# husheng876/pytorch_nested-unet

Hardware: AMD Instinct MI355X
Metric: images/sec NestedUNet 96x96 bs=16 train (higher is better)
Workload: dtype bf16; 1 GPU; NestedUNet(num_classes=1, in=3, deep_supervision=False) 96x96 per-GPU batch 16, bf16 storage / fp32 accumulate, BCEDiceLoss, SGD(1e-3, 0.9, wd 1e-4), fwd+loss+iou+bwd+sgd per step (BASELINE.json configs[1]); global_batch=16, parallelism=dp1, hip_graph=True

## Files before the change

### include/nunet_diag.h

```cpp
#ifndef NUNET_DIAG_H
#define NUNET_DIAG_H

#include "nunet.h"

#ifdef __cplusplus
extern "C" {
#endif

int nunet_plan_set_lanes(nunet_plan* p, nunet_stream_t* lanes, int32_t n);
int nunet_plan_stamps_read(nunet_plan* plan, int32_t pass, uint64_t* ticks, int32_t cap, int32_t* n_out, char* labels, int32_t label_bytes);
int nunet_debug_stamp(uint64_t* dst, nunet_stream_t stream);
int nunet_debug_spin(int32_t us, int32_t tag, nunet_stream_t stream);

typedef struct {
  int32_t tile;
  int32_t BM, BN, HPMAX, NT;
  int32_t NI, TH, TW, SH;
  int32_t tilesX, tilesY, tilesG;
  int32_t nCoT;
  int32_t S, nch;
  int32_t items;
  int32_t grid;
  int32_t per_cu;
} nunet_conv_launch_info;
int nunet_conv3x3_launch_info(const nunet_conv_desc* d, nunet_conv_launch_info* out);

typedef struct {
  int32_t A, B;
  int32_t NI, TH, TW, SH;
  int32_t tilesX, tilesY, tilesG;
  int32_t nMT;
  int32_t nCoT, nCiT;
  int32_t ksplit;
  int32_t grid;
} nunet_wgrad_launch_info;
int nunet_conv3x3_wgrad_launch_info(const nunet_wgrad_desc* d, nunet_wgrad_launch_info* out);

#ifdef __cplusplus
}
#endif
#endif
```

### pytorch_nested-unet_amd/_lib.py

```python
import ctypes as C
import os
import subprocess

import torch

_HERE = os.path.dirname(os.path.abspath(__file__))
LIB_PATH = os.environ.get("NUNET_LIB_PATH") or os.path.join(_HERE, "libnunet.so")

F32, BF16, F16 = 0, 1, 2
DTYPES = {"fp32": F32, "float32": F32, "bf16": BF16, "bfloat16": BF16, "fp16": F16, "float16": F16,
          torch.float32: F32, torch.bfloat16: BF16, torch.float16: F16}
TORCH_DTYPE = {F32: torch.float32, BF16: torch.bfloat16, F16: torch.float16}

_vp, _i32, _i64, _u32, _f32, _sz = C.c_void_p, C.c_int32, C.c_int64, C.c_uint32, C.c_float, C.c_size_t
BN_SUM_REPLICAS = 8
FX_WORDS = 2
TF_NONE, TF_BN_RELU, TF_BN_RELU_BWD = 0, 1, 2


def fx_zeros(c, device):
    return torch.zeros(BN_SUM_REPLICAS * 2 * c * FX_WORDS, dtype=torch.int64, device=device)


def fx_decode(buf, c):
# ... 9 lines not shown
    buf[0, :, 0] = hi.to(torch.int64)
    buf[0, :, 1] = lo.to(torch.int64)
    return buf.reshape(-1).to(device)


class ConvDesc(C.Structure):
    _fields_ = [("dtype", _i32), ("N", _i32), ("H", _i32), ("W", _i32),
                ("src0", _vp), ("C0", _i32), ("P0", _i32),
                ("src1", _vp), ("C1", _i32), ("P1", _i32),
                ("wpack", _vp), ("bias", _vp),
                ("dst0", _vp), ("D0", _i32), ("Q0", _i32),
                ("dst1", _vp), ("D1", _i32), ("Q1", _i32),
                ("acc_slot_w", _i32), ("acc0_mask", _u32), ("acc1", _i32),
                ("stats", _vp), ("splitk_ws", _vp), ("splitk_ws_floats", _i64),
                ("bn_y", _vp), ("bn_py", _i32), ("bn_mean_invstd", _vp), ("bn_gamma", _vp), ("bn_beta", _vp), ("bn_sums", _vp),
                ("in_tf", _i32), ("tf_training", _i32), ("tf_y", _vp), ("tf_py", _i32), ("tf_fx", _vp),
                ("tf_gamma", _vp), ("tf_beta", _vp), ("tf_conv_bias", _vp),
                ("tf_running_mean", _vp), ("tf_running_var", _vp), ("tf_nbt", _vp), ("tf_mean_invstd", _vp),
                ("tf_momentum", _f32), ("tf_eps", _f32),
                ("tf_dgamma", _vp), ("tf_dbeta", _vp), ("tf_dbias", _vp), ("tf_store", _vp), ("tf_ps", _i32), ("tile", _i32)]


class WgradDesc(C.Structure):
    _fields_ = [("dtype", _i32), ("N", _i32), ("H", _i32), ("W", _i32),
                ("src0", _vp), ("C0", _i32), ("P0", _i32),
                ("src1", _vp), ("C1", _i32), ("P1", _i32),
                ("dy", _vp), ("Cout", _i32), ("PY", _i32),
                ("dw", _vp), ("slab_stride", _i64), ("max_slabs", _i32), ("target_wgs", _i32), ("dw_floats", _i64), ("item_shape", _i32)]


class ConvLaunchInfo(C.Structure):
    _fields_ = [(k, _i32) for k in ("tile", "BM", "BN", "HPMAX", "NT", "NI", "TH", "TW", "SH", "tilesX", "tilesY", "tilesG",
                                    "nCoT", "S", "nch", "items", "grid", "per_cu")]


class WgradLaunchInfo(C.Structure):
    _fields_ = [(k, _i32) for k in ("A", "B", "NI", "TH", "TW", "SH", "tilesX", "tilesY", "tilesG", "nMT", "nCoT", "nCiT",
                                    "ksplit", "grid")]


class BnFwdDesc(C.Structure):
    _fields_ = [("dtype", _i32), ("N", _i32), ("H", _i32), ("W", _i32), ("C", _i32),
                ("y", _vp), ("PY", _i32),
                ("conv_bias", _vp), ("stats", _vp), ("gamma", _vp), ("beta", _vp),
                ("running_mean", _vp), ("running_var", _vp), ("num_batches_tracked", _vp),
                ("save_mean_invstd", _vp),
                ("training", _i32), ("momentum", _f32), ("eps", _f32),
                ("a", _vp), ("PA", _i32), ("pooled", _vp), ("PP", _i32), ("up", _vp), ("PU", _i32)]


class BnBwdDesc(C.Structure):
    _fields_ = [("dtype", _i32), ("N", _i32), ("H", _i32), ("W", _i32), ("C", _i32),
                ("da", _vp), ("PDA", _i32), ("y", _vp), ("PY", _i32),
                ("mean_invstd", _vp), ("gamma", _vp), ("beta", _vp),
                ("sums", _vp), ("dgamma", _vp), ("dbeta", _vp), ("dbias", _vp),
                ("dy", _vp), ("PDY", _i32)]


class BnrDesc(C.Structure):
    _fields_ = [("y", _vp), ("PY", _i32), ("mean_invstd", _vp), ("gamma", _vp), ("beta", _vp), ("sums", _vp)]


class ProfEntry(C.Structure):
    _fields_ = [("name", C.c_char * 48), ("launches", _i32), ("ms", C.c_double), ("flops", C.c_double),
                ("bytes", C.c_double)]

# ... 64 lines not shown
    "nunet_nchw_to_nhwc": (_i32, [_vp, _i32, _i32, _i32, _i32, _i32, _vp, _i32, _vp]),
    "nunet_plan_create": (_vp, [C.POINTER(PlanCfg)]),
    "nunet_plan_destroy": (None, [_vp]),
    "nunet_plan_arena_bytes": (C.c_size_t, [_vp]),
    "nunet_plan_param_count": (_i64, [_vp]),
    "nunet_plan_bnbuf_count": (_i64, [_vp]),
    "nunet_plan_bn_layers": (_i32, [_vp]),
    "nunet_plan_num_heads": (_i32, [_vp]),
    "nunet_plan_forward": (_i32, [_vp, _vp, _vp, _vp, _vp, _vp, _sz, _vp, _i32, _vp]),
    "nunet_plan_stage_u8": (_i32, [_vp, _vp, _vp, _vp, _vp, _f32, _vp, _sz, _vp]),
    "nunet_plan_backward": (_i32, [_vp, _vp, _vp, _vp, _sz, _vp, _i32, _vp]),
    "nunet_plan_backward_phase": (_i32, [_vp, _vp, _vp, _vp, _sz, _vp, _i32, _i32, _vp]),
    "nunet_plan_grad_scratch": (_i32, [_vp, C.POINTER(_i64), C.POINTER(_i64), C.POINTER(_i64)]),
    "nunet_plan_bucket0_enable": (_i32, [_vp, _i32]),
    "nunet_plan_bucket0_wait": (_i32, [_vp, _vp]),
    "nunet_plan_opt_step": (_i32, [_vp, _vp, C.POINTER(Optim), _vp, _sz, _f32, _vp, _i32, _vp]),
    "nunet_plan_set_inpass_opt": (_i32, [_vp, _vp, C.POINTER(Optim), _f32, _vp]),
    "nunet_plan_grad_sqnorm_ws_bytes": (C.c_size_t, [_vp]),
    "nunet_plan_grad_sqnorm": (_i32, [_vp, _vp, _sz, _vp, _sz, _vp]),
    "nunet_plan_repack": (_i32, [_vp, _vp, _vp, _sz, _vp]),
    "nunet_plan_feature": (_i64, [_vp, _i32, _i32, C.POINTER(_i32), C.POINTER(_i32)]),
    "nunet_plan_set_multistream": (_i32, [_vp, _i32]),
    "nunet_plan_set_schedule": (_i32, [_vp, _i32]),
    "nunet_plan_calibrate": (_i32, [_vp, _i32]),
    "nunet_plan_set_lane_priority": (_i32, [_vp, _i32]),
    "nunet_plan_reset_lanes": (_i32, [_vp]),
    "nunet_plan_set_lanes": (_i32, [_vp, C.POINTER(_vp), _i32]),
    "nunet_profile_begin": (_i32, []),
    "nunet_profile_end": (_i32, [C.POINTER(ProfEntry), _i32, C.POINTER(_i32)]),
    "nunet_debug_spin": (_i32, [_i32, _i32, _vp]),
    "nunet_debug_stamp": (_i32, [_vp, _vp]),
    "nunet_conv3x3_launch_info": (_i32, [C.POINTER(ConvDesc), C.POINTER(ConvLaunchInfo)]),
    "nunet_conv3x3_wgrad_launch_info": (_i32, [C.POINTER(WgradDesc), C.POINTER(WgradLaunchInfo)]),
    "nunet_graph_begin": (_i32, [_vp]),
    "nunet_graph_end": (_i32, [_vp, C.POINTER(_vp)]),
    "nunet_graph_launch": (_i32, [_vp, _vp]),
    "nunet_graph_info": (_i32, [_vp, C.POINTER(_i32), C.POINTER(_i32), C.POINTER(_i32)]),
    "nunet_graph_destroy": (None, [_vp]),
    "nunet_seg_begin": (_i32, [_vp, _i32]),
    "nunet_seg_end": (_i32, [_vp, C.POINTER(_vp)]),
    "nunet_seg_launch": (_i32, [_vp, _vp]),
    "nunet_seg_info": (_i32, [_vp, C.POINTER(_i32), C.POINTER(_i32), C.POINTER(_i32), C.POINTER(_i32)]),
    "nunet_seg_destroy": (None, [_vp]),
    "nunet_plan_stamps_read": (_i32, [_vp, _i32, C.POINTER(C.c_uint64), _i32, C.POINTER(_i32), C.c_char_p, _i32]),
}

_lib = None


class NunetError(RuntimeError):
    pass


def build(verbose=False):
    cmd = ["make", "-C", os.path.join(_HERE, "csrc"), "-j4"]
    r = subprocess.run(cmd, capture_output=True, text=True)
    if r.returncode != 0:
        raise NunetError("building libnunet.so failed:\n" + r.stdout + r.stderr)
    if verbose:
        print(r.stdout)
    return LIB_PATH


def lib():
    global _lib
    if _lib is None:
# ... 54 lines not shown
```

### pytorch_nested-unet_amd/csrc/conv3x3.hip

```cpp
#include <stdlib.h>
#include <type_traits>

#include "common.h"

template <typename T> struct Mma;
template <> struct Mma<bf16_t> {
  typedef bf16x8 Frag;
  static __device__ __forceinline__ Frag load(const bf16_t* p) { return *reinterpret_cast<const bf16x8*>(p); }
  static __device__ __forceinline__ void mma(f32x16& acc, const Frag& a, const Frag& b) {
    acc = __builtin_amdgcn_mfma_f32_32x32x16_bf16(a, b, acc, 0, 0, 0);
  }
  static __device__ __forceinline__ void sink(const Frag& a) { asm volatile("" :: "v"(a)); }
};
template <> struct Mma<f16_t> {
  typedef f16x8 Frag;
  static __device__ __forceinline__ Frag load(const f16_t* p) { return *reinterpret_cast<const f16x8*>(p); }
  static __device__ __forceinline__ void mma(f32x16& acc, const Frag& a, const Frag& b) {
    acc = __builtin_amdgcn_mfma_f32_32x32x16_f16(a, b, acc, 0, 0, 0);
  }
  static __device__ __forceinline__ void sink(const Frag& a) { asm volatile("" :: "v"(a)); }
};
template <> struct Mma<float> {
  struct Frag { f32x4 lo, hi; };
  static __device__ __forceinline__ Frag load(const float* p) {
// ... 111 lines not shown
#define KSTAMP_RT(i) do {} while (0)
#endif

#ifndef NUNET_ABLATE
#define NUNET_ABLATE 0
#endif

static inline int conv_coef_floats(int lt, int cin, bool bnr, int cout) { return (lt == 1 ? 2 : lt == 2 ? 4 : 0) * cin + (bnr ? 4 * cout : 0) + cout; }

struct ConvGroup { int n; int grid[CONV_GROUP_MAX]; ConvP p[CONV_GROUP_MAX]; };

#ifndef NUNET_XCD_REMAP
#define NUNET_XCD_REMAP 1
#endif
__device__ __forceinline__ int xcd_remap(int b, int G) {
  if (!NUNET_XCD_REMAP) return b;
  const int x = b & 7, l = b >> 3, q = G >> 3, rem = G & 7;
  return (x < rem ? x * (q + 1) : rem * (q + 1) + (x - rem) * q) + l;
}
__device__ __forceinline__ void conv_group_decode(const ConvGroup& g, int b, int& k, int& v) {
  int base = 0, prevg = 0, live = g.n;
  k = 0; v = b;
#pragma unroll
  for (int j = 0; j < CONV_GROUP_MAX; ++j) {
    if (j < g.n) {
      const int span = (g.grid[j] - prevg) * live;
      if (b >= base && b < base + span) { const int r = b - base; const int q = r / live; k = j + (r - q * live); v = prevg + q; }
      base += span; prevg = g.grid[j]; --live;
    }
  }
}

template <typename T, int WM, int WN, int SM, int SN, bool SK, bool BNR, int LT>
__global__ __launch_bounds__(64 * WM * WN, 2) void conv3x3_kernel(ConvGroup grp) {
  typedef ConvCfg<T, WM, WN, SM, SN> C;
  int gk = 0, vbid = (int)blockIdx.x;
  if (grp.n > 1) conv_group_decode(grp, (int)blockIdx.x, gk, vbid);
  gk = __builtin_amdgcn_readfirstlane(gk); vbid = __builtin_amdgcn_readfirstlane(vbid);
  const ConvP& p = grp.p[gk];
  const int vgrid = grp.grid[gk];
  typedef Mma<T> M;
  constexpr int PS = C::PS, EPV = C::EPV, BN = C::BN, BM = C::BM, NT = C::NT, KS = C::KS, OS = C::OS;

  __shared__ __attribute__((aligned(16))) T s_buf[C::STAGE_ELEMS];
  __shared__ int s_hidx[BM];
  __shared__ int s_mxy[BM];
  __shared__ int s_hxy[C::HPMAX];
  __shared__ int s_gpix[BM];
  __shared__ float s_red[2 * WM * BN];
  extern __shared__ __attribute__((aligned(16))) float s_coef[];
  T* const s_halo = s_buf;
  T* const s_w = s_buf + C::HALO_ELEMS;
  float* const s_bnc = s_coef + (LT == 1 ? 2 : LT == 2 ? 4 : 0) * p.Cin;
  float* const s_bias = s_bnc + (BNR ? 4 : 0) * p.Cout;

  const int tid = threadIdx.x, lane = tid & 63, wave = tid >> 6;
  const int wm = wave / WN, wn = wave % WN;
  const int r = lane & 31, h = lane >> 5;
  const int HW2 = p.TW + 2, HH2 = p.TH + 2;
  const int HP = p.NI * HH2 * HW2;
  const int THW = p.TH * p.TW;
  KSTAMP(0); KSTAMP_RT(30);
  [[maybe_unused]] int kst = 4;

  for (int m = tid; m < BM; m += NT) {
    const int r32 = m & 31;
    const int q = (r32 < 4) ? r32 : (r32 < 12) ? r32 + 12 : (r32 < 16) ? r32 - 8 : (r32 < 20) ? r32 + 8 : (r32 < 28) ? r32 - 12 : r32;
    const int t = (m & ~31) + q;
    const int ni = fastdiv(t, p.invTHW);
    const int rem = t - ni * THW;
    const int ly = fastdiv(rem, p.invTW), lx = rem - ly * p.TW;
    const bool ok = ni < p.NI;
    s_hidx[m] = ok ? ((ni * HH2 + ly + 1) * HW2 + lx + 1) : (HW2 + 1);
    s_mxy[m] = ok ? ((ni << 20) | (ly << 10) | lx) : -1;
  }
  for (int hp = tid; hp < C::HPMAX; hp += NT) {
    int code = -1;
    if (hp < HP) {
      const int ni = fastdiv(hp, p.invHH2HW2);
      const int rem = hp - ni * (HH2 * HW2);
      const int hy = fastdiv(rem, p.invHW2), hx = rem - hy * HW2;
      code = (ni << 20) | (hy << 10) | hx;
    }
    s_hxy[hp] = code;
  }
  __syncthreads();
  KSTAMP(1);

  int abase[SM];
#pragma unroll
  for (int a = 0; a < SM; ++a) abase[a] = s_hidx[(wm * SM + a) * 32 + r] * PS + 8 * h;
  int toff[9];
#pragma unroll
  for (int tap = 0; tap < 9; ++tap) toff[tap] = ((tap / 3 - 1) * HW2 + (tap % 3 - 1)) * PS;
  const int bbase = ((wn * SN) * 32 + r) * PS + 8 * h;
  int hcode[C::UH];
  unsigned interior = 0u;
#pragma unroll
  for (int k = 0; k < C::UH; ++k) {
    const int hp = (tid + k * NT) >> 2;
    hcode[k] = hp < C::HPMAX ? s_hxy[hp] : -1;
    if (LT != 0 && hcode[k] >= 0) {
      const int hy = (hcode[k] >> 10) & 1023, hx = hcode[k] & 1023;
      if (hy >= 1 && hy <= p.TH && hx >= 1 && hx <= p.TW) interior |= 1u << k;
    }
  }
  const int seg = tid & 3;

  struct Item { int co0, n0, y0, x0, ks; };
  auto decode = [&](int item) {
    Item it;
    it.ks = 0;
    if constexpr (SK) { const int q = fastdiv(item, p.invS); it.ks = item - q * p.S; item = q; }
    int q = fastdiv(item, p.invCoT);
    it.co0 = (item - q * p.nCoT) * BN; item = q;
    q = fastdiv(item, p.invTX);
    it.x0 = (item - q * p.tilesX) * p.TW; item = q;
    q = fastdiv(item, p.invTY);
    it.y0 = (item - q * p.tilesY) * p.TH;
    it.n0 = q * p.NI;
    return it;
  };

  int hgp[C::UH];
  auto set_hgp = [&](const Item& it) {
#pragma unroll
    for (int k = 0; k < C::UH; ++k) {
      int gp = -1;
      if (hcode[k] >= 0) {
        const int n = it.n0 + (hcode[k] >> 20), y = it.y0 + ((hcode[k] >> 10) & 1023) - 1, x = it.x0 + (hcode[k] & 1023) - 1;
        gp = map_pixel(n, y, x, p.N, p.H, p.W, p.SH, p.SHinv);
      }
      hgp[k] = gp;
    }
  };

  Vec16<T> hreg[C::UH];
  Vec16<T> yreg[LT == 2 ? C::UH : 1];
  Vec16<T> wreg[C::UW];
  unsigned woff[C::UW];
#pragma unroll
  for (int k = 0; k < C::UW; ++k) {
    const int u = tid + k * NT;
    const int row = u >> 2;
    const int tap = row / BN, co = row - tap * BN;
    woff[k] = row < 9 * BN ? (unsigned)(((tap * p.Cout + co) * p.Cin + seg * EPV) * (int)sizeof(T)) : (unsigned)(seg * 16);
  }
  unsigned wco = 0u;
  auto set_ptrs = [&](const Item& it) { wco = (unsigned)(it.co0 * p.Cin * (int)sizeof(T)); };
  struct LoadCtx { const char* base; unsigned pb, cb, yb, ycb, wb; };
  auto load_ctx = [&](int kb) {
    LoadCtx c;
    const bool s0 = LT != 0 || kb < p.C0;
    c.base = (const char*)(s0 ? p.src0 : p.src1);
    c.pb = (unsigned)(s0 ? p.P0 : p.P1) * (unsigned)sizeof(T);
    c.cb = (unsigned)((s0 ? kb : kb - p.C0) * (int)sizeof(T) + seg * 16);
    c.yb = (unsigned)p.tf_py * (unsigned)sizeof(T);
    c.ycb = (unsigned)(kb * (int)sizeof(T) + seg * 16);
    c.wb = (unsigned)(kb * (int)sizeof(T)) + wco;
    return c;
  };
  constexpr int NU = C::UH + C::UW;
  auto load_unit = [&](const LoadCtx& c, int u) {
    if (u < C::UH) {
      const unsigned gp = hgp[u] < 0 ? 0u : (unsigned)hgp[u];
      hreg[u].raw = *reinterpret_cast<const u32x4*>(c.base + (gp * c.pb + c.cb));
      if constexpr (LT == 2) yreg[u].raw = *reinterpret_cast<const u32x4*>((const char*)p.tf_y + (gp * c.yb + c.ycb));
    } else {
      wreg[u - C::UH].raw = *reinterpret_cast<const u32x4*>((const char*)p.w + (woff[u - C::UH] + c.wb));
    }
  };
  auto load_regs = [&](int kb) {
    const LoadCtx c = load_ctx(kb);
#pragma unroll
    for (int u = 0; u < NU; ++u) load_unit(c, u);
  };
  auto write_lds = [&](int kb, bool store) {
    if constexpr (LT == 0) {
#pragma unroll
      for (int k = 0; k < C::UH; ++k) {
        const int u = tid + k * NT;
        if ((k + 1) * NT <= C::HPMAX * 4 || (u >> 2) < C::HPMAX) st16(&s_halo[(u >> 2) * PS + seg * EPV], hgp[k] >= 0 ? hreg[k] : zero16<T>());
      }
    } else {
      typedef typename FV<T>::type V;
      const int c0 = kb + seg * EPV;
      const V sc = ldf<T>(&s_coef[c0]), sh = ldf<T>(&s_coef[p.Cin + c0]);
      V cA, cB;
      if constexpr (LT == 2) { cA = ldf<T>(&s_coef[2 * p.Cin + c0]); cB = ldf<T>(&s_coef[3 * p.Cin + c0]); }
#pragma unroll
      for (int k = 0; k < C::UH; ++k) {
        const int u = tid + k * NT;
        if ((k + 1) * NT <= C::HPMAX * 4 || (u >> 2) < C::HPMAX) {
          const bool ok = hgp[k] >= 0;
          V v;
          if constexpr (LT == 1) v = bn_relu_apply<V>(vec_to_f<T>(hreg[k]), sc, sh);
          else v = bn_relu_bwd_apply<V>(vec_to_f<T>(hreg[k]), vec_to_f<T>(yreg[k]), sc, sh, cA, cB);
          Vec16<T> o = vec_from_f<T>(v);
          if (!ok) o = zero16<T>();
          st16(&s_halo[(u >> 2) * PS + seg * EPV], o);
          if (store && ok && ((interior >> k) & 1u)) st16((T*)p.tf_store + (size_t)hgp[k] * p.tf_ps + c0, o);
        }
      }
    }
#pragma unroll
    for (int k = 0; k < C::UW; ++k) {
      const int u = tid + k * NT;
      if ((k + 1) * NT <= 9 * BN * 4 || (u >> 2) < 9 * BN) st16(&s_w[(u >> 2) * PS + seg * EPV], wreg[k]);
    }
  };

  f32x16 acc[SM][SN];
#pragma unroll
  for (int a = 0; a < SM; ++a)
#pragma unroll
    for (int b = 0; b < SN; ++b)
#pragma unroll
      for (int i = 0; i < 16; ++i) acc[a][b][i] = 0.f;

  auto chunk_kb = [&](int c) { return c < p.nch0 ? c * C::KC : p.C0 + (c - p.nch0) * C::KC; };
  constexpr int NSTEP = 9 * KS;
  auto sweep = [&](auto LOADS, const LoadCtx& lc) {
    constexpr bool WITH_LOADS = decltype(LOADS)::value;
    constexpr int PD = 1;
    constexpr int NB = PD + 1;
    typename M::Frag fa[NB][SM], fb[NB][SN];
    auto read_step = [&](int j) {
      const int tap = j / KS, ks = j % KS, bu = j % NB;
#pragma unroll
      for (int a = 0; a < SM; ++a) fa[bu][a] = M::load(&s_halo[abase[a] + toff[tap] + ks * 16]);
#pragma unroll
      for (int b = 0; b < SN; ++b) fb[bu][b] = M::load(&s_w[bbase + (tap * BN + b * 32) * PS + ks * 16]);
    };
#pragma unroll
    for (int j = 0; j < PD; ++j) read_step(j);
#pragma unroll
    for (int j = 0; j < NSTEP; ++j) {
      if (j + PD < NSTEP && !(NUNET_ABLATE & 2)) read_step(j + PD);
      if constexpr (WITH_LOADS && !(NUNET_ABLATE & 4)) {
#pragma unroll
        for (int u = 0; u < NU; ++u)
          if ((u * NSTEP) / NU == j) load_unit(lc, u);
      }
      __builtin_amdgcn_sched_barrier(0);
#pragma unroll
      for (int a = 0; a < SM; ++a)
#pragma unroll
        for (int b = 0; b < SN; ++b) {
          if constexpr (NUNET_ABLATE & 1) { M::sink(fa[j % NB][a]); M::sink(fb[j % NB][b]); }
          else M::mma(acc[a][b], fa[j % NB][a], fb[j % NB][b]);
        }
      __builtin_amdgcn_sched_barrier(0);
    }
  };
  auto epi_sk = [&](const Item& cur) {
    float* slab = p.slabs + (size_t)cur.ks * p.slab_stride;
#pragma unroll
    for (int b = 0; b < SN; ++b) {
      const int co = cur.co0 + (wn * SN + b) * 32 + r;
#pragma unroll
      for (int a = 0; a < SM; ++a) {
#pragma unroll
        for (int i = 0; i < 16; ++i) {
          const int gp = s_gpix[(wm * SM + a) * 32 + acc_row(i, h)];
          if (gp >= 0) slab[(size_t)gp * p.Cout + co] = acc[a][b][i];
          acc[a][b][i] = 0.f;
        }
      }
    }
  };
  static_assert(SM * 16 <= 64, "row-validity mask of the epilogue is one 64-bit word");
  Vec16<T> byv[BNR ? C::UO : 1];
  auto issue_byv = [&](const Item& cur) {
    if constexpr (BNR) {
      constexpr int SEGS = BN / EPV;
      const int sg = tid % SEGS, m0 = tid / SEGS;
#pragma unroll
      for (int k = 0; k < C::UO; ++k) {
        const int m = m0 + k * (NT / SEGS);
        const int gp = m < BM ? s_gpix[m] : -1;
        byv[k] = ld16((const T*)p.bn_y + (size_t)(gp < 0 ? 0 : gp) * p.bn_py + cur.co0 + sg * EPV);
      }
    }
  };
  auto epi_plain = [&](const Item& cur, T* const s_out) {
    constexpr int SEGS = BN / EPV;
    const int sg = tid % SEGS, m0 = tid / SEGS;
    int gpu[C::UO];
#pragma unroll
    for (int k = 0; k < C::UO; ++k) {
      const int m = m0 + k * (NT / SEGS);
      gpu[k] = m < BM ? s_gpix[m] : -1;
    }
    unsigned long long rowmask = 0ull;
    if (p.stats) {
#pragma unroll
      for (int a = 0; a < SM; ++a)
#pragma unroll
        for (int i = 0; i < 16; ++i) rowmask |= (s_gpix[(wm * SM + a) * 32 + acc_row(i, h)] >= 0 ? 1ull : 0ull) << (a * 16 + i);
    }
    KSTAMP(kst); ++kst;
    __syncthreads();
    KSTAMP(kst); ++kst;
#pragma unroll
    for (int b = 0; b < SN; ++b) {
      const int cl = (wn * SN + b) * 32 + r;
      const float bias = s_bias[cur.co0 + cl];
      float s1 = 0.f, s2 = 0.f;
#pragma unroll
      for (int a = 0; a < SM; ++a) {
#pragma unroll
        for (int i = 0; i < 16; ++i) {
          const int m = (wm * SM + a) * 32 + acc_row(i, h);
          const T tv = from_f32<T>(acc[a][b][i] + bias);
          if (!(NUNET_ABLATE & 1024)) s_out[m * OS + cl] = tv;
          const float d = ((rowmask >> (a * 16 + i)) & 1ull) ? to_f32(tv) - bias : 0.f;
          s1 += d; s2 += d * d;
          acc[a][b][i] = 0.f;
        }
      }
      if (p.stats) {
        s1 += __shfl_xor(s1, 32);
        s2 += __shfl_xor(s2, 32);
        if (h == 0) { s_red[(wm * BN + cl) * 2 + 0] = s1; s_red[(wm * BN + cl) * 2 + 1] = s2; }
      }
    }
    KSTAMP(kst); ++kst;
    __syncthreads();
    KSTAMP(kst); ++kst;
    typedef typename FV<T>::type V;
    V bmean, bistd, bsc, bsh, r1 = V(0.f), r2 = V(0.f);
    if constexpr (BNR) {
      const int c0 = cur.co0 + sg * EPV;
      bmean = ldf<T>(&s_bnc[c0]); bistd = ldf<T>(&s_bnc[p.Cout + c0]); bsc = ldf<T>(&s_bnc[2 * p.Cout + c0]); bsh = ldf<T>(&s_bnc[3 * p.Cout + c0]);
    }
    const int co = cur.co0 + sg * EPV;
    const bool to0 = co < p.D0;
    T* const qb = to0 ? (T*)p.dst0 + co : (T*)p.dst1 + (co - p.D0);
    const int qs = to0 ? __builtin_amdgcn_readfirstlane(p.Q0) : __builtin_amdgcn_readfirstlane(p.Q1);
    const bool accum = to0 ? ((p.acc0_mask >> (p.slot_w > 0 ? fastdiv(co, p.inv_slot_w) : 0)) & 1u) != 0u : p.acc1 != 0;
    const bool any_accum = p.acc0_mask != 0u || p.acc1 != 0;
    Vec16<T> vv[C::UO];
#pragma unroll
    for (int k = 0; k < C::UO; ++k) {
      const int m = m0 + k * (NT / SEGS);
      vv[k] = ld16(&s_out[(m < BM ? m : 0) * OS + sg * EPV]);
    }
#pragma unroll
    for (int k = 0; k < C::UO; ++k) {
// ... 54 lines not shown
  Item cur = decode(item);
  set_hgp(cur);
  set_ptrs(cur);
  int cc = 0, c_hi = 0;
  int kb = 0;
  if constexpr (SK) { cc = cur.ks * p.nch / p.S; c_hi = (cur.ks + 1) * p.nch / p.S; kb = chunk_kb(cc); }
  KSTAMP(2);
  load_regs(kb);
  bool first_chunk = true;
  for (int c = tid; c < p.Cout; c += NT) s_bias[c] = p.bias ? p.bias[c] : 0.f;
  if constexpr (BNR) {
    for (int c = tid; c < p.Cout; c += NT) {
      const float mean = p.bn_mi[c], istd = p.bn_mi[p.Cout + c];
      const float sc = p.bn_gamma[c] * istd;
      s_bnc[c] = mean; s_bnc[p.Cout + c] = istd; s_bnc[2 * p.Cout + c] = sc; s_bnc[3 * p.Cout + c] = __builtin_fmaf(-mean, sc, p.bn_beta[c]);
    }
  }
  if constexpr (LT == 1) {
    BnStatArgs a; a.fx = p.tf_fx; a.conv_bias = p.tf_bias; a.rm = p.tf_rm; a.rv = p.tf_rv; a.C = p.Cin; a.training = p.tf_training; a.M = p.M; a.eps = p.tf_eps;
    for (int c = tid; c < p.Cin; c += NT) {
      float mean, invstd, var, mf;
      bn_stat_coeffs(a, c, mean, invstd, var, mf);
      const float sc = p.tf_gamma[c] * invstd;
      s_coef[c] = sc; s_coef[p.Cin + c] = __builtin_fmaf(-mean, sc, p.tf_beta[c]);
      if (vbid == 0 && p.tf_training) {
        if (p.tf_save) { p.tf_save[c] = mean; p.tf_save[p.Cin + c] = invstd; }
        if (p.tf_rm) bn_running_update(p.tf_rm, p.tf_rv, c, p.tf_momentum, mf, var, p.M);
      }
    }
    if (vbid == 0 && p.tf_training && tid == 0 && p.tf_nbt) *p.tf_nbt += 1;
  }
  if constexpr (LT == 2) {
    const int nrep = bn_sum_replicas(p.Cin);
    for (int c = tid; c < p.Cin; c += NT) {
      const float mean = p.tf_save[c], istd = p.tf_save[p.Cin + c];
      const float sc = p.tf_gamma[c] * istd;
      double t1, t2;
      fx_totals(p.tf_fx, p.Cin, nrep, c, t1, t2);
      float A, B;
      bn_bwd_AB(mean, istd, sc, (float)(t1 / (double)p.M), (float)(t2 / (double)p.M), A, B);
      s_coef[c] = sc; s_coef[p.Cin + c] = __builtin_fmaf(-mean, sc, p.tf_beta[c]); s_coef[2 * p.Cin + c] = A; s_coef[3 * p.Cin + c] = B;
      if (vbid == 0) {
        if (p.tf_dbeta) p.tf_dbeta[c] = (float)t1;
        if (p.tf_dgamma) p.tf_dgamma[c] = (float)t2;
        if (p.tf_dbias) p.tf_dbias[c] = 0.f;
      }
    }
  }

  KSTAMP(3);
  while (true) {
    __syncthreads();
    KSTAMP(kst); ++kst;
    if (!(NUNET_ABLATE & 8) || (item == vbid && first_chunk)) write_lds(kb, LT != 0 && p.tf_store != nullptr && cur.co0 == 0);
    KSTAMP(kst); ++kst;
    if (first_chunk) {
      for (int m = tid; m < BM; m += NT) {
        const int code = s_mxy[m];
        int gp = -1;
        if (code >= 0) {
          const int n = cur.n0 + (code >> 20), y = cur.y0 + ((code >> 10) & 1023), x = cur.x0 + (code & 1023);
          gp = map_pixel(n, y, x, p.N, p.H, p.W, p.SH, p.SHinv);
        }
        s_gpix[m] = gp;
      }
    }
    __syncthreads();
    KSTAMP(kst); ++kst;
    int nkb = kb + C::KC, nitem = item, ncc = cc + 1, nc_hi = c_hi;
    Item nxt = cur;
    bool have_next = true;
    bool last_chunk;
    if constexpr (SK) last_chunk = ncc >= c_hi; else last_chunk = nkb >= p.Cin;
    if (last_chunk) {
      nkb = 0;
      nitem = item + vgrid;
      if (nitem < p.nItems) {
        nxt = decode(nitem); set_hgp(nxt); set_ptrs(nxt);
// ... 122 lines not shown
      if (nimax > N) nimax = N;
      for (int ni = 1; ni <= nimax; ++ni) {
        const long hp = (long)ni * (th + 2) * (tw + 2);
        if (hp > HPMAX) continue;
        const int tX = ceil_div(W, tw), tY = ceil_div(H, th), tG = ceil_div(N, ni);
        const double util = (double)N * H * W / ((double)tX * tY * tG * BM);
        const double halo = (double)hp / ((double)ni * th * tw);
        const double score = util * 1000.0 - halo * 10.0 + (tw >= 16 ? 1.0 : 0.0);
        if (score > best_score) { best_score = score; best = TileGeom{ni, th, tw, tX, tY, tG, 0}; }
      }
    }
  }
  if (W <= BM && (long)N * (H + 1) < (1 << 20) && H + 1 <= 4096) {
    const double best_util = (double)N * H * W / ((double)best.tilesX * best.tilesY * best.tilesG * BM);
    const int VH = N * (H + 1);
    double su = 0.0; int sth = 0;
    for (int th = 1; th * W <= BM && th < 1000; ++th) {
      if ((long)(th + 2) * (W + 2) > HPMAX) break;
      const int tY = ceil_div(VH, th);
      const double util = (double)N * H * W / ((double)tY * BM);
      if (util > su) { su = util; sth = th; }
    }
    if (sth > 0 && su > best_util * 1.08) best = TileGeom{1, sth, W, 1, ceil_div(VH, sth), 1, H + 1};
  }
  return best;
}

template <typename T, int WM, int WN, int SM, int SN, bool SK, bool BNR>
static void launch_conv_lt(int lt, unsigned grid, size_t dyn, hipStream_t st, const ConvGroup& g) {
  typedef ConvCfg<T, WM, WN, SM, SN> C;
  if (lt == 1) NUNET_LAUNCH((conv3x3_kernel<T, WM, WN, SM, SN, SK, BNR, 1>), dim3(grid), dim3(C::NT), dyn, st, g);
  else if (lt == 2) NUNET_LAUNCH((conv3x3_kernel<T, WM, WN, SM, SN, SK, BNR, 2>), dim3(grid), dim3(C::NT), dyn, st, g);
  else NUNET_LAUNCH((conv3x3_kernel<T, WM, WN, SM, SN, SK, BNR, 0>), dim3(grid), dim3(C::NT), dyn, st, g);
}

struct ConvSetup { ConvP p; long grid; long per_cu; size_t dyn; bool bnr; int lt; double flops, bytes; };
template <typename T, int WM, int WN, int SM, int SN>
static void conv_setup(const nunet_conv_desc* d, ConvSetup& S) {
  typedef ConvCfg<T, WM, WN, SM, SN> C;
  ConvP& p = S.p;
  p.src0 = d->src0; p.src1 = d->src1; p.C0 = d->C0; p.C1 = d->C1; p.P0 = d->P0; p.P1 = d->P1;
  p.w = d->wpack; p.bias = d->bias;
  p.dst0 = d->dst0; p.dst1 = d->dst1; p.D0 = d->D0; p.D1 = d->D1; p.Q0 = d->Q0; p.Q1 = d->Q1;
  p.slot_w = d->acc_slot_w; p.acc0_mask = d->acc0_mask; p.acc1 = d->acc1; p.inv_slot_w = fastdiv_inv(d->acc_slot_w);
  p.stats = (long long*)d->stats;
  p.N = d->N; p.H = d->H; p.W = d->W; p.Cin = d->C0 + d->C1; p.Cout = d->D0 + d->D1;
  p.M = (float)d->N * d->H * d->W;
  const bool bnr = d->bn_y != nullptr;
  const int lt = d->in_tf;
  p.bn_y = d->bn_y; p.bn_py = d->bn_py; p.bn_mi = d->bn_mean_invstd; p.bn_gamma = d->bn_gamma; p.bn_beta = d->bn_beta; p.bn_sums = (long long*)d->bn_sums;
  p.tf_y = d->tf_y; p.tf_py = d->tf_py; p.tf_fx = (const long long*)d->tf_fx; p.tf_gamma = d->tf_gamma; p.tf_beta = d->tf_beta; p.tf_bias = d->tf_conv_bias;
  p.tf_rm = d->tf_running_mean; p.tf_rv = d->tf_running_var; p.tf_nbt = (long long*)d->tf_nbt; p.tf_save = d->tf_mean_invstd;
  p.tf_training = d->tf_training; p.tf_momentum = d->tf_momentum; p.tf_eps = d->tf_eps;
  p.tf_dgamma = d->tf_dgamma; p.tf_dbeta = d->tf_dbeta; p.tf_dbias = d->tf_dbias; p.tf_store = d->tf_store; p.tf_ps = d->tf_ps;
  const TileGeom g = nunet_choose_tile(d->N, d->H, d->W, C::BM, C::HPMAX);
  p.NI = g.NI; p.TH = g.TH; p.TW = g.TW; p.tilesX = g.tilesX; p.tilesY = g.tilesY; p.tilesG = g.tilesG; p.SH = g.SH;
  p.SHinv = g.SH ? (unsigned)(((1ull << 32) + g.SH - 1) / g.SH) : 0u;
  p.nCoT = p.Cout / C::BN;
  long items = (long)p.nCoT * g.tilesX * g.tilesY * g.tilesG;
  p.S = 1; p.slabs = nullptr; p.slab_stride = 0;
  p.nch0 = p.C0 / C::KC;
  p.nch = p.nch0 + p.C1 / C::KC;
#ifndef NUNET_SK_ITEMS
#define NUNET_SK_ITEMS 60
#define NUNET_SK_TARGET 320
#endif
  if (d->splitk_ws && items <= NUNET_SK_ITEMS && p.nch >= 8 && p.Cout <= 1024 && (256 / (p.Cout / C::EPV)) >= 1) {
    int Sn = (int)((NUNET_SK_TARGET + items - 1) / items);
    if (Sn > p.nch / 2) Sn = p.nch / 2;
    const long long need = (long long)Sn * d->N * d->H * d->W * p.Cout;
    if (Sn > 1 && need <= d->splitk_ws_floats) {
      p.S = Sn; p.slabs = d->splitk_ws; p.slab_stride = (long long)d->N * d->H * d->W * p.Cout;
      items *= Sn;
    }
  }
  p.nItems = (int)items;
  p.invS = fastdiv_inv(p.S); p.invCoT = fastdiv_inv(p.nCoT); p.invTX = fastdiv_inv(p.tilesX); p.invTY = fastdiv_inv(p.tilesY);
  p.invTHW = fastdiv_inv(g.TH * g.TW); p.invTW = fastdiv_inv(g.TW); p.invHH2HW2 = fastdiv_inv((g.TH + 2) * (g.TW + 2)); p.invHW2 = fastdiv_inv(g.TW + 2);
  S.bnr = bnr; S.lt = lt;
  S.dyn = sizeof(float) * (size_t)conv_coef_floats(lt, p.Cin, bnr && p.S == 1, p.Cout);
  const size_t lds_bytes = sizeof(T) * C::STAGE_ELEMS + 4 * (3 * C::BM + C::HPMAX) + 8 * WM * C::BN + S.dyn;
  long per_cu = (long)(160 * 1024 / lds_bytes);
  if (per_cu < 1) per_cu = 1;
  if (per_cu > 2048 / C::NT) per_cu = 2048 / C::NT;
  S.per_cu = per_cu;
  const long resident = 256 * per_cu;
  const long rounds = (items + resident - 1) / resident;
  S.grid = (items + rounds - 1) / rounds;
  const double px = (double)d->N * d->H * d->W;
  const int acin = g_prof_alg_cin > 0 ? g_prof_alg_cin : p.Cin;
  S.flops = 2.0 * 9 * acin * p.Cout * px;
  S.bytes = (px * (acin * (lt == 2 ? 2 : 1) + p.Cout) + 9.0 * acin * p.Cout) * sizeof(T);
}

template <typename T, int WM, int WN, int SM, int SN>
static int launch_conv_cfg(const nunet_conv_desc* d, hipStream_t st) {
  typedef ConvCfg<T, WM, WN, SM, SN> C;
  ConvSetup s0;
  conv_setup<T, WM, WN, SM, SN>(d, s0);
  const ConvP& p = s0.p;
  const int cls = C::BN == 64 ? PC_CONV_M128N64 : C::BM == 256 ? PC_CONV_M256N32 : PC_CONV_M128N32;
  ProfScope ps(cls, s0.flops, s0.bytes, st);
  ConvGroup g; g.n = 1; g.grid[0] = (int)s0.grid; g.p[0] = p;
  if (p.S > 1) {
    launch_conv_lt<T, WM, WN, SM, SN, true, false>(s0.lt, (unsigned)s0.grid, s0.dyn, st, g);
    SplitFinP f;
    f.slabs = p.slabs; f.slab_stride = p.slab_stride; f.S = p.S; f.bias = p.bias;
    f.dst0 = p.dst0; f.dst1 = p.dst1; f.D0 = p.D0; f.D1 = p.D1; f.Q0 = p.Q0; f.Q1 = p.Q1;
    f.slot_w = p.slot_w; f.acc0_mask = p.acc0_mask; f.acc1 = p.acc1; f.inv_slot_w = p.inv_slot_w; f.stats = p.stats;
    f.npix = (long long)d->N * d->H * d->W; f.Cout = p.Cout;
    f.bn_y = p.bn_y; f.bn_py = p.bn_py; f.bn_mi = p.bn_mi; f.bn_gamma = p.bn_gamma; f.bn_beta = p.bn_beta; f.bn_sums = p.bn_sums;
    const int G = p.Cout / C::EPV;
    const int blk = G * (256 / G);
    long long fg = (f.npix + (blk / G) - 1) / (blk / G);
    if (fg > 1024) fg = 1024;
    if (s0.bnr) NUNET_LAUNCH((splitk_finalize_kernel<T, true>), dim3((unsigned)fg), dim3(blk), 0, st, f);
    else NUNET_LAUNCH((splitk_finalize_kernel<T, false>), dim3((unsigned)fg), dim3(blk), 0, st, f);
// ... 64 lines not shown
}
extern "C" int nunet_conv3x3_fwd(const nunet_conv_desc* d, nunet_stream_t s) {
  const int rc = conv_check(d);
  if (rc) return rc;
  return NUNET_DISPATCH(d->dtype, launch_conv, d, (hipStream_t)s);
}

template <typename T, int WM, int WN, int SM, int SN>
static int conv_info_cfg(const nunet_conv_desc* d, int cfg, nunet_conv_launch_info* o) {
  typedef ConvCfg<T, WM, WN, SM, SN> C;
  ConvSetup S;
  conv_setup<T, WM, WN, SM, SN>(d, S);
  const ConvP& p = S.p;
  o->tile = cfg + 1; o->BM = C::BM; o->BN = C::BN; o->HPMAX = C::HPMAX; o->NT = C::NT;
  o->NI = p.NI; o->TH = p.TH; o->TW = p.TW; o->SH = p.SH;
  o->tilesX = p.tilesX; o->tilesY = p.tilesY; o->tilesG = p.tilesG; o->nCoT = p.nCoT;
  o->S = p.S; o->nch = p.nch; o->items = p.nItems; o->grid = (int32_t)S.grid; o->per_cu = (int32_t)S.per_cu;
  return NUNET_OK;
}
template <typename T> static int conv_info(const nunet_conv_desc* d, nunet_conv_launch_info* o) {
  const int cfg = conv_cfg_of(d);
  if (cfg == 0) return conv_info_cfg<T, 4, 1, 1, 1>(d, cfg, o);
  if (cfg == 1) return conv_info_cfg<T, 2, 2, 2, 1>(d, cfg, o);
  if (cfg == 3) return conv_info_cfg<T, 4, 1, 2, 2>(d, cfg, o);
  return conv_info_cfg<T, 4, 1, 2, 1>(d, cfg, o);
}
extern "C" int nunet_conv3x3_launch_info(const nunet_conv_desc* d, nunet_conv_launch_info* out) {
  NUNET_REQUIRE(out, "conv3x3 launch info: null output");
  const int rc = conv_check(d, false);
  if (rc) return rc;
  return NUNET_DISPATCH(d->dtype, conv_info, d, out);
}

struct WgP {
  const void* src0; const void* src1;
  int C0, C1, P0, P1;
  const void* dy; int Cout, PY;
  float* dw; long long slab_stride;
  int N, H, W, Cin;
  int NI, TH, TW, tilesX, tilesY, tilesG;
  int nCoT, nCiT, ksplit, nMT;
  int SH; unsigned SHinv;
  unsigned invTX, invTY;
};

template <typename T, int A_, int B_> struct WgCfg {
  static constexpr int A = A_, B = B_;
  static constexpr int NT = 192;
  static constexpr int BM = 128, HPMAX = 192;
  static constexpr int EPV = Tr<T>::EPV;
  static constexpr bool F32 = std::is_same<T, float>::value;
  static constexpr int SR = 32;
  static constexpr int UPR = 32 / EPV;
  static constexpr int UPD = UPR * A, UPX = UPR * B;
  static constexpr int NUD = (BM * UPD + NT - 1) / NT;
  static constexpr int NUA = (HPMAX * UPX + NT - 1) / NT;
  static constexpr int STAGE = (BM * A + HPMAX * B) * SR;
  static_assert(NT % UPD == 0 && NT % UPX == 0, "every staging unit of a thread has the same channel segment");
  static_assert(NUD <= 16 && NUA <= 32, "validity masks");
};

template <typename T>
__device__ __forceinline__ s16x4 tr_read(const T* p) {
  return __builtin_amdgcn_ds_read_tr16_b64_v4i16(
      (__attribute__((address_space(3))) s16x4*)(const_cast<T*>(p)));
}
// ... 439 lines not shown
```

Baseline: 9566 images/sec.

## Raise conv3x3 occupancy to three workgroups per CU for single-subtile configs

Sets launch bounds to three workgroups per CU for conv configs with SM*SN==1, and caps the persistent grid's per-CU count at that value. To fit the tighter register budget it also cuts live registers: per-row A offsets replace the abase/toff arrays, a computed weight offset replaces the woff array, and the epilogue recomputes thread indices. The LT==2 BN-backward coefficient prologue now reduces the replicated fixed-point sums through LDS instead of each thread looping over replicas. The tighter register cap may cause spills, and a kernel-attributes query is added for diagnostics.

```diff
diff --git a/include/nunet_diag.h b/include/nunet_diag.h
--- a/include/nunet_diag.h
+++ b/include/nunet_diag.h
@@ -26,6 +26,16 @@
 int nunet_conv3x3_launch_info(const nunet_conv_desc* d, nunet_conv_launch_info* out);
 
 typedef struct {
+  int32_t numRegs;
+  int32_t localSizeBytes;
+  int32_t sharedSizeBytes;
+  int32_t blockSize, dynLdsBytes;
+  int32_t occupancy;
+  int32_t wg_per_cu;
+} nunet_conv_kernel_attrs_t;
+int nunet_conv_kernel_attrs(const nunet_conv_desc* d, nunet_conv_kernel_attrs_t* out);
+
+typedef struct {
   int32_t A, B;
   int32_t NI, TH, TW, SH;
   int32_t tilesX, tilesY, tilesG;
diff --git a/pytorch_nested-unet_amd/_lib.py b/pytorch_nested-unet_amd/_lib.py
--- a/pytorch_nested-unet_amd/_lib.py
+++ b/pytorch_nested-unet_amd/_lib.py
@@ -65,6 +65,11 @@
 class ConvLaunchInfo(C.Structure):
     _fields_ = [(k, _i32) for k in ("tile", "BM", "BN", "HPMAX", "NT", "NI", "TH", "TW", "SH", "tilesX", "tilesY", "tilesG",
                                     "nCoT", "S", "nch", "items", "grid", "per_cu")]
+
+
+class ConvKernelAttrs(C.Structure):
+    _fields_ = [(k, _i32) for k in ("numRegs", "localSizeBytes", "sharedSizeBytes", "blockSize", "dynLdsBytes", "occupancy",
+                                    "wg_per_cu")]
 
 
 class WgradLaunchInfo(C.Structure):
@@ -195,6 +200,7 @@
     "nunet_debug_stamp": (_i32, [_vp, _vp]),
     "nunet_conv3x3_launch_info": (_i32, [C.POINTER(ConvDesc), C.POINTER(ConvLaunchInfo)]),
     "nunet_conv3x3_wgrad_launch_info": (_i32, [C.POINTER(WgradDesc), C.POINTER(WgradLaunchInfo)]),
+    "nunet_conv_kernel_attrs": (_i32, [C.POINTER(ConvDesc), C.POINTER(ConvKernelAttrs)]),
     "nunet_graph_begin": (_i32, [_vp]),
     "nunet_graph_end": (_i32, [_vp, C.POINTER(_vp)]),
     "nunet_graph_launch": (_i32, [_vp, _vp]),
diff --git a/pytorch_nested-unet_amd/csrc/conv3x3.hip b/pytorch_nested-unet_amd/csrc/conv3x3.hip
--- a/pytorch_nested-unet_amd/csrc/conv3x3.hip
+++ b/pytorch_nested-unet_amd/csrc/conv3x3.hip
@@ -167,7 +167,13 @@
 }
 
 template <typename T, int WM, int WN, int SM, int SN, bool SK, bool BNR, int LT>
-__global__ __launch_bounds__(64 * WM * WN, 2) void conv3x3_kernel(ConvGroup grp) {
+constexpr int conv_wg_per_cu() {
+  if (SM * SN > 1) return 2;
+  return 3;
+}
+
+template <typename T, int WM, int WN, int SM, int SN, bool SK, bool BNR, int LT>
+__global__ __launch_bounds__(64 * WM * WN, (conv_wg_per_cu<T, WM, WN, SM, SN, SK, BNR, LT>())) void conv3x3_kernel(ConvGroup grp) {
   typedef ConvCfg<T, WM, WN, SM, SN> C;
   int gk = 0, vbid = (int)blockIdx.x;
   if (grp.n > 1) conv_group_decode(grp, (int)blockIdx.x, gk, vbid);
@@ -176,6 +182,7 @@
   const int vgrid = grp.grid[gk];
   typedef Mma<T> M;
   constexpr int PS = C::PS, EPV = C::EPV, BN = C::BN, BM = C::BM, NT = C::NT, KS = C::KS, OS = C::OS;
+  static_assert(NT == 256, "four waves per workgroup on every tile");
 
   __shared__ __attribute__((aligned(16))) T s_buf[C::STAGE_ELEMS];
   __shared__ int s_hidx[BM];
@@ -222,12 +229,11 @@
   __syncthreads();
   KSTAMP(1);
 
-  int abase[SM];
-#pragma unroll
-  for (int a = 0; a < SM; ++a) abase[a] = s_hidx[(wm * SM + a) * 32 + r] * PS + 8 * h;
-  int toff[9];
-#pragma unroll
-  for (int tap = 0; tap < 9; ++tap) toff[tap] = ((tap / 3 - 1) * HW2 + (tap % 3 - 1)) * PS;
+  int arow[SM][3];
+#pragma unroll
+  for (int a = 0; a < SM; ++a)
+#pragma unroll
+    for (int ty = 0; ty < 3; ++ty) arow[a][ty] = (s_hidx[(wm * SM + a) * 32 + r] + (ty - 1) * HW2 - 1) * PS + 8 * h;
   const int bbase = ((wn * SN) * 32 + r) * PS + 8 * h;
   int hcode[C::UH];
   unsigned interior = 0u;
@@ -241,6 +247,7 @@
     }
   }
   const int seg = tid & 3;
+  const int srow = (tid >> 2) * PS + seg * EPV;
 
   struct Item { int co0, n0, y0, x0, ks; };
   auto decode = [&](int item) {
@@ -273,14 +280,9 @@
   Vec16<T> hreg[C::UH];
   Vec16<T> yreg[LT == 2 ? C::UH : 1];
   Vec16<T> wreg[C::UW];
-  unsigned woff[C::UW];
-#pragma unroll
-  for (int k = 0; k < C::UW; ++k) {
-    const int u = tid + k * NT;
-    const int row = u >> 2;
-    const int tap = row / BN, co = row - tap * BN;
-    woff[k] = row < 9 * BN ? (unsigned)(((tap * p.Cout + co) * p.Cin + seg * EPV) * (int)sizeof(T)) : (unsigned)(seg * 16);
-  }
+  static_assert((NT / 4) % BN == 0, "weight staging units of a thread differ by whole taps");
+  const unsigned woff0 = (unsigned)(((((tid >> 2) / BN) * p.Cout + (tid >> 2) % BN) * p.Cin + seg * EPV) * (int)sizeof(T));
+  const unsigned wstep = (unsigned)((NT / 4 / BN) * p.Cout * p.Cin * (int)sizeof(T));
   unsigned wco = 0u;
   auto set_ptrs = [&](const Item& it) { wco = (unsigned)(it.co0 * p.Cin * (int)sizeof(T)); };
   struct LoadCtx { const char* base; unsigned pb, cb, yb, ycb, wb; };
@@ -302,7 +304,10 @@
       hreg[u].raw = *reinterpret_cast<const u32x4*>(c.base + (gp * c.pb + c.cb));
       if constexpr (LT == 2) yreg[u].raw = *reinterpret_cast<const u32x4*>((const char*)p.tf_y + (gp * c.yb + c.ycb));
     } else {
-      wreg[u - C::UH].raw = *reinterpret_cast<const u32x4*>((const char*)p.w + (woff[u - C::UH] + c.wb));
+      const int k = u - C::UH;
+      unsigned wo = woff0 + (unsigned)k * wstep;
+      if ((k + 1) * NT > 9 * BN * 4 && (tid >> 2) + k * (NT / 4) >= 9 * BN) wo = (unsigned)(seg * 16);
+      wreg[k].raw = *reinterpret_cast<const u32x4*>((const char*)p.w + (wo + c.wb));
     }
   };
   auto load_regs = [&](int kb) {
@@ -315,7 +320,7 @@
 #pragma unroll
       for (int k = 0; k < C::UH; ++k) {
         const int u = tid + k * NT;
-        if ((k + 1) * NT <= C::HPMAX * 4 || (u >> 2) < C::HPMAX) st16(&s_halo[(u >> 2) * PS + seg * EPV], hgp[k] >= 0 ? hreg[k] : zero16<T>());
+        if ((k + 1) * NT <= C::HPMAX * 4 || (u >> 2) < C::HPMAX) st16(&s_halo[srow + k * (NT / 4) * PS], hgp[k] >= 0 ? hreg[k] : zero16<T>());
       }
     } else {
       typedef typename FV<T>::type V;
@@ -333,7 +338,7 @@
           else v = bn_relu_bwd_apply<V>(vec_to_f<T>(hreg[k]), vec_to_f<T>(yreg[k]), sc, sh, cA, cB);
           Vec16<T> o = vec_from_f<T>(v);
           if (!ok) o = zero16<T>();
-          st16(&s_halo[(u >> 2) * PS + seg * EPV], o);
+          st16(&s_halo[srow + k * (NT / 4) * PS], o);
           if (store && ok && ((interior >> k) & 1u)) st16((T*)p.tf_store + (size_t)hgp[k] * p.tf_ps + c0, o);
         }
       }
@@ -341,7 +346,7 @@
 #pragma unroll
     for (int k = 0; k < C::UW; ++k) {
       const int u = tid + k * NT;
-      if ((k + 1) * NT <= 9 * BN * 4 || (u >> 2) < 9 * BN) st16(&s_w[(u >> 2) * PS + seg * EPV], wreg[k]);
+      if ((k + 1) * NT <= 9 * BN * 4 || (u >> 2) < 9 * BN) st16(&s_w[srow + k * (NT / 4) * PS], wreg[k]);
     }
   };
 
@@ -360,10 +365,14 @@
     constexpr int PD = 1;
     constexpr int NB = PD + 1;
     typename M::Frag fa[NB][SM], fb[NB][SN];
+#pragma unroll
+    for (int a = 0; a < SM; ++a)
+#pragma unroll
+      for (int ty = 0; ty < 3; ++ty) asm volatile("" : "+v"(arow[a][ty]));
     auto read_step = [&](int j) {
       const int tap = j / KS, ks = j % KS, bu = j % NB;
 #pragma unroll
-      for (int a = 0; a < SM; ++a) fa[bu][a] = M::load(&s_halo[abase[a] + toff[tap] + ks * 16]);
+      for (int a = 0; a < SM; ++a) fa[bu][a] = M::load(&s_halo[arow[a][tap / 3] + (tap % 3) * PS + ks * 16]);
 #pragma unroll
       for (int b = 0; b < SN; ++b) fb[bu][b] = M::load(&s_w[bbase + (tap * BN + b * 32) * PS + ks * 16]);
     };
@@ -404,12 +413,13 @@
       }
     }
   };
-  static_assert(SM * 16 <= 64, "row-validity mask of the epilogue is one 64-bit word");
   Vec16<T> byv[BNR ? C::UO : 1];
   auto issue_byv = [&](const Item& cur) {
     if constexpr (BNR) {
       constexpr int SEGS = BN / EPV;
-      const int sg = tid % SEGS, m0 = tid / SEGS;
+      int tid_e = threadIdx.x;
+      asm volatile("" : "+v"(tid_e));
+      const int sg = tid_e % SEGS, m0 = tid_e / SEGS;
 #pragma unroll
       for (int k = 0; k < C::UO; ++k) {
         const int m = m0 + k * (NT / SEGS);
@@ -420,6 +430,11 @@
   };
   auto epi_plain = [&](const Item& cur, T* const s_out) {
     constexpr int SEGS = BN / EPV;
+    int tid_e = threadIdx.x;
+    asm volatile("" : "+v"(tid_e));
+    const int tid = tid_e, lane = tid & 63, wave = tid >> 6;
+    const int wm = wave / WN, wn = wave % WN;
+    const int r = lane & 31, h = lane >> 5;
     const int sg = tid % SEGS, m0 = tid / SEGS;
     int gpu[C::UO];
 #pragma unroll
@@ -427,12 +442,14 @@
       const int m = m0 + k * (NT / SEGS);
       gpu[k] = m < BM ? s_gpix[m] : -1;
     }
-    unsigned long long rowmask = 0ull;
+    unsigned rowmask[SM];
+#pragma unroll
+    for (int a = 0; a < SM; ++a) rowmask[a] = 0u;
     if (p.stats) {
 #pragma unroll
       for (int a = 0; a < SM; ++a)
 #pragma unroll
-        for (int i = 0; i < 16; ++i) rowmask |= (s_gpix[(wm * SM + a) * 32 + acc_row(i, h)] >= 0 ? 1ull : 0ull) << (a * 16 + i);
+        for (int i = 15; i >= 0; --i) rowmask[a] = (rowmask[a] << 1) | (s_gpix[(wm * SM + a) * 32 + acc_row(i, h)] >= 0 ? 1u : 0u);
     }
     KSTAMP(kst); ++kst;
     __syncthreads();
@@ -449,7 +466,7 @@
           const int m = (wm * SM + a) * 32 + acc_row(i, h);
           const T tv = from_f32<T>(acc[a][b][i] + bias);
           if (!(NUNET_ABLATE & 1024)) s_out[m * OS + cl] = tv;
-          const float d = ((rowmask >> (a * 16 + i)) & 1ull) ? to_f32(tv) - bias : 0.f;
+          const float d = ((rowmask[a] >> i) & 1u) ? to_f32(tv) - bias : 0.f;
           s1 += d; s2 += d * d;
           acc[a][b][i] = 0.f;
         }
@@ -570,18 +587,39 @@
   }
   if constexpr (LT == 2) {
     const int nrep = bn_sum_replicas(p.Cin);
-    for (int c = tid; c < p.Cin; c += NT) {
-      const float mean = p.tf_save[c], istd = p.tf_save[p.Cin + c];
-      const float sc = p.tf_gamma[c] * istd;
-      double t1, t2;
-      fx_totals(p.tf_fx, p.Cin, nrep, c, t1, t2);
+    auto finish = [&](int c, float mean, float istd, float gam, float bet, const fx2_t& q0, const fx2_t& q1) {
+      const float sc = gam * istd;
+      const double t1 = fx_value(q0[0], q0[1]), t2 = fx_value(q1[0], q1[1]);
       float A, B;
       bn_bwd_AB(mean, istd, sc, (float)(t1 / (double)p.M), (float)(t2 / (double)p.M), A, B);
-      s_coef[c] = sc; s_coef[p.Cin + c] = __builtin_fmaf(-mean, sc, p.tf_beta[c]); s_coef[2 * p.Cin + c] = A; s_coef[3 * p.Cin + c] = B;
+      s_coef[c] = sc; s_coef[p.Cin + c] = __builtin_fmaf(-mean, sc, bet); s_coef[2 * p.Cin + c] = A; s_coef[3 * p.Cin + c] = B;
       if (vbid == 0) {
         if (p.tf_dbeta) p.tf_dbeta[c] = (float)t1;
         if (p.tf_dgamma) p.tf_dgamma[c] = (float)t2;
         if (p.tf_dbias) p.tf_dbias[c] = 0.f;
+      }
+    };
+    if (nrep > 1) {
+      fx2_t* const s_fx = reinterpret_cast<fx2_t*>(s_buf);
+      const bool own = tid < p.Cin;
+      float mean = 0.f, istd = 0.f, gam = 0.f, bet = 0.f;
+      if (own) { mean = p.tf_save[tid]; istd = p.tf_save[p.Cin + tid]; gam = p.tf_gamma[tid]; bet = p.tf_beta[tid]; }
+      if (tid < nrep * p.Cin) {
+        const int rr = tid / p.Cin, c = tid - rr * p.Cin;
+#pragma unroll
+        for (int v = 0; v < 2; ++v) s_fx[tid * 2 + v] = *reinterpret_cast<const fx2_t*>(p.tf_fx + ((size_t)(rr * 2 + v) * p.Cin + c) * NUNET_FX_WORDS);
+      }
+      __syncthreads();
+      if (own) {
+        fx2_t q0 = s_fx[tid * 2], q1 = s_fx[tid * 2 + 1];
+        for (int rr = 1; rr < nrep; ++rr) { q0 += s_fx[(rr * p.Cin + tid) * 2]; q1 += s_fx[(rr * p.Cin + tid) * 2 + 1]; }
+        finish(tid, mean, istd, gam, bet, q0, q1);
+      }
+    } else {
+      for (int c = tid; c < p.Cin; c += NT) {
+        const fx2_t q0 = *reinterpret_cast<const fx2_t*>(p.tf_fx + (size_t)c * NUNET_FX_WORDS);
+        const fx2_t q1 = *reinterpret_cast<const fx2_t*>(p.tf_fx + (size_t)(p.Cin + c) * NUNET_FX_WORDS);
+        finish(c, p.tf_save[c], p.tf_save[p.Cin + c], p.tf_gamma[c], p.tf_beta[c], q0, q1);
       }
     }
   }
@@ -770,6 +808,20 @@
   if (lt == 1) NUNET_LAUNCH((conv3x3_kernel<T, WM, WN, SM, SN, SK, BNR, 1>), dim3(grid), dim3(C::NT), dyn, st, g);
   else if (lt == 2) NUNET_LAUNCH((conv3x3_kernel<T, WM, WN, SM, SN, SK, BNR, 2>), dim3(grid), dim3(C::NT), dyn, st, g);
   else NUNET_LAUNCH((conv3x3_kernel<T, WM, WN, SM, SN, SK, BNR, 0>), dim3(grid), dim3(C::NT), dyn, st, g);
+}
+
+struct ConvKernelRef { int wg_per_cu; const void* fn; };
+template <typename T, int WM, int WN, int SM, int SN, bool SK, bool BNR>
+static ConvKernelRef conv_kernel_ref_lt(int lt) {
+  if (lt == 1) return {conv_wg_per_cu<T, WM, WN, SM, SN, SK, BNR, 1>(), (const void*)conv3x3_kernel<T, WM, WN, SM, SN, SK, BNR, 1>};
+  if (lt == 2) return {conv_wg_per_cu<T, WM, WN, SM, SN, SK, BNR, 2>(), (const void*)conv3x3_kernel<T, WM, WN, SM, SN, SK, BNR, 2>};
+  return {conv_wg_per_cu<T, WM, WN, SM, SN, SK, BNR, 0>(), (const void*)conv3x3_kernel<T, WM, WN, SM, SN, SK, BNR, 0>};
+}
+template <typename T, int WM, int WN, int SM, int SN>
+static ConvKernelRef conv_kernel_ref(bool sk, bool bnr, int lt) {
+  if (sk) return conv_kernel_ref_lt<T, WM, WN, SM, SN, true, false>(lt);
+  if (bnr) return conv_kernel_ref_lt<T, WM, WN, SM, SN, false, true>(lt);
+  return conv_kernel_ref_lt<T, WM, WN, SM, SN, false, false>(lt);
 }
 
 struct ConvSetup { ConvP p; long grid; long per_cu; size_t dyn; bool bnr; int lt; double flops, bytes; };
@@ -821,6 +873,8 @@
   long per_cu = (long)(160 * 1024 / lds_bytes);
   if (per_cu < 1) per_cu = 1;
   if (per_cu > 2048 / C::NT) per_cu = 2048 / C::NT;
+  const long by_regs = conv_kernel_ref<T, WM, WN, SM, SN>(p.S > 1, bnr, lt).wg_per_cu;
+  if (per_cu > by_regs) per_cu = by_regs;
   S.per_cu = per_cu;
   const long resident = 256 * per_cu;
   const long rounds = (items + resident - 1) / resident;
@@ -951,6 +1005,36 @@
   return NUNET_DISPATCH(d->dtype, conv_info, d, out);
 }
 
+template <typename T, int WM, int WN, int SM, int SN>
+static int conv_attrs_cfg(const nunet_conv_desc* d, nunet_conv_kernel_attrs_t* o) {
+  typedef ConvCfg<T, WM, WN, SM, SN> C;
+  ConvSetup S;
+  conv_setup<T, WM, WN, SM, SN>(d, S);
+  const ConvKernelRef k = conv_kernel_ref<T, WM, WN, SM, SN>(S.p.S > 1, S.bnr, S.lt);
+  hipFuncAttributes a;
+  hipError_t e = hipFuncGetAttributes(&a, k.fn);
+  NUNET_REQUIRE(e == hipSuccess, "conv3x3 kernel attrs: hipFuncGetAttributes: %s", hipGetErrorString(e));
+  int occ = 0;
+  e = hipOccupancyMaxActiveBlocksPerMultiprocessor(&occ, k.fn, C::NT, S.dyn);
+  NUNET_REQUIRE(e == hipSuccess, "conv3x3 kernel attrs: hipOccupancyMaxActiveBlocksPerMultiprocessor: %s", hipGetErrorString(e));
+  o->numRegs = a.numRegs; o->localSizeBytes = (int32_t)a.localSizeBytes; o->sharedSizeBytes = (int32_t)a.sharedSizeBytes;
+  o->blockSize = C::NT; o->dynLdsBytes = (int32_t)S.dyn; o->occupancy = occ; o->wg_per_cu = k.wg_per_cu;
+  return NUNET_OK;
+}
+template <typename T> static int conv_attrs(const nunet_conv_desc* d, nunet_conv_kernel_attrs_t* o) {
+  const int cfg = conv_cfg_of(d);
+  if (cfg == 0) return conv_attrs_cfg<T, 4, 1, 1, 1>(d, o);
+  if (cfg == 1) return conv_attrs_cfg<T, 2, 2, 2, 1>(d, o);
+  if (cfg == 3) return conv_attrs_cfg<T, 4, 1, 2, 2>(d, o);
+  return conv_attrs_cfg<T, 4, 1, 2, 1>(d, o);
+}
+extern "C" int nunet_conv_kernel_attrs(const nunet_conv_desc* d, nunet_conv_kernel_attrs_t* out) {
+  NUNET_REQUIRE(out, "conv3x3 kernel attrs: null output");
+  const int rc = conv_check(d, false);
+  if (rc) return rc;
+  return NUNET_DISPATCH(d->dtype, conv_attrs, d, out);
+}
+
 struct WgP {
   const void* src0; const void* src1;
   int C0, C1, P0, P1;
```

Result: faster. 9676 images/sec (median of 6 runs) (+1.2%).
